# vani-nag/OWLRayTracing

Hardware: AMD Instinct MI355X
Metric: kNN queries/sec (10M pts, k=10) (higher is better)
Workload: dtype f32; 1 GPU; TrueKNN on 10000000 uniform-random 3-D points (numpy default_rng(0), [0,1)^3), k=10, start radius 0.25*(k/n)^(1/3)=0.0025; BASELINE.json configs[1]; ranks=1, n_points_total=10000000, k=10, kernel=team_kernel, parallelism=1 GPU

## Files before the change

owlraytracing_amd/csrc/lbvh.h:

```cpp
#pragma once
#include <hip/hip_runtime.h>
#include <stdint.h>

#include <string>

#include "owl/lbvh_device.h"

#define LBVH_PATH_BLOCK 64
#define LBVH_PATH_WORDS 5

namespace owlmi {

struct HipError {
  std::string what;
};
struct LbvhStateError : HipError {};

#define OWLMI_HIP(call)                                                                        \
  do {                                                                                         \
    hipError_t e_ = (call);                                                                    \
    if (e_ != hipSuccess)                                                                      \
      throw ::owlmi::HipError{std::string(#call) + " failed: " + hipGetErrorString(e_) + " (" + \
                              __FILE__ + ":" + std::to_string(__LINE__) + ")"};                \
  } while (0)

class Lbvh {
 public:
  Lbvh() = default;
  ~Lbvh();
  Lbvh(const Lbvh &) = delete;
  Lbvh &operator=(const Lbvh &) = delete;

  void build_from_points(const float *d_xyz, int64_t n, hipStream_t stream, const int32_t *d_ids = nullptr, const int32_t *d_batch = nullptr,
                         int batch_bits = 0);
  void build_from_boxes(const LbvhBox *d_boxes, int64_t n, hipStream_t stream);
  void refit_boxes(const LbvhBox *d_boxes, hipStream_t stream);

  LbvhView view() const;
  LbvhWideView wide_view() const;
  const float *scene_device() const { return scene_; }
  int32_t *nan_count() const { return reinterpret_cast<int32_t *>(scene_ + 6); }
  const int32_t *split_owner_device() const { return split_owner_; }
  const int32_t *block_paths_device() const { return point_mode_ && n_ > 1 ? block_paths_ : nullptr; }
  const int32_t *row_slot_device() const { return point_mode_ && built_ ? reinterpret_cast<const int32_t *>(order_) : nullptr; }
  const uint64_t *keys_device() const { return built_ ? codes_alt_ : nullptr; }
  int curve() const { return curve_; }
  int64_t size() const { return n_; }
  bool built() const { return built_; }
  void clear() { built_ = false; }
  bool has_points() const { return points_ != nullptr && point_mode_; }
  size_t device_bytes() const { return bytes_; }

  void download(LbvhNode *nodes, int32_t *rope_node, int32_t *rope_leaf, int32_t *prim_id,
                hipStream_t stream) const;
  void download_tables(int32_t *split_owner, int32_t *block_paths, hipStream_t stream) const;
  struct DebugInfo {
    int32_t curve, nan_count, wide_levels, wide_count[LBVH_WIDE_LEVELS];
    float scene[6];
  };
  int64_t sentinel_end() const { return (n_ + LBVH_BLOCK - 1) / LBVH_BLOCK * LBVH_BLOCK + LBVH_BLOCK; }
  void download_debug(DebugInfo *info, uint64_t *keys, LbvhPoint *points, int32_t *row_slot, LbvhBox *wide_boxes,
                      int64_t wide_capacity, hipStream_t stream) const;
  void download_boxes(LbvhBox *sorted_boxes, hipStream_t stream) const;

 private:
  void reserve(int64_t n);
  void release();
  void sort_and_tree(hipStream_t stream);
  void fit(hipStream_t stream);

  int64_t n_ = 0, cap_ = 0;
  bool built_ = false, point_mode_ = false;
  int curve_ = 0;
  size_t bytes_ = 0;
// ... 21 lines not shown
```

owlraytracing_amd/csrc/lbvh.hip:

```cpp
#include "lbvh.h"

#include "curve_key.h"

#include <hipcub/hipcub.hpp>

#include <cstdlib>
#include <cstring>

namespace owlmi {
namespace {

constexpr int kPartialBlocks = 1024;
constexpr int kBlock = 256;

struct Box6 {
  float lo[3], hi[3];
};

__device__ __forceinline__ Box6 empty_box() {
  Box6 b;
  b.lo[0] = b.lo[1] = b.lo[2] = INFINITY;
  b.hi[0] = b.hi[1] = b.hi[2] = -INFINITY;
  return b;
}
// ... 165 lines not shown
  nodes[i].other = (int32_t)j;
  split_owner[gamma] = (int32_t)i;
}

template <int SRC>
__global__ void __launch_bounds__(kBlock) table_kernel(const void *__restrict__ in, int64_t n_in,
                                                      LbvhBox *__restrict__ out, int64_t n_out) {
  int64_t j = ((int64_t)blockIdx.x * kBlock + threadIdx.x) >> 6;
  if (j >= n_out) return;
  int64_t i = j * 64 + (threadIdx.x & 63);
  Box6 b = empty_box();
  if (i < n_in) {
    if (SRC == 0) {
      LbvhPoint p = ((const LbvhPoint *)in)[i];
      float c[3] = {p.x, p.y, p.z};
      grow(b, c, c);
    } else {
      LbvhBox q = ((const LbvhBox *)in)[i];
      grow(b, q.lo, q.hi);
    }
  }
  b = wave_union(b);
  if ((threadIdx.x & 63) == 0) {
    LbvhBox o;
    for (int a = 0; a < 3; a++) {
      o.lo[a] = b.lo[a];
      o.hi[a] = b.hi[a];
    }
    out[j] = o;
  }
}

__global__ void __launch_bounds__(kBlock) block_box_kernel(const LbvhPoint *__restrict__ pts, int64_t n,
                                                          LbvhBox *__restrict__ out, int64_t n_out) {
  int64_t b = (int64_t)blockIdx.x * kBlock + threadIdx.x;
  if (b >= n_out) return;
  Box6 box = empty_box();
  for (int j = 0; j < LBVH_BLOCK; j++) {
    int64_t i = b * LBVH_BLOCK + j;
    if (i < n) {
      LbvhPoint p = pts[i];
      float c[3] = {p.x, p.y, p.z};
      grow(box, c, c);
    }
  }
  LbvhBox o;
  for (int a = 0; a < 3; a++) {
    o.lo[a] = box.lo[a];
    o.hi[a] = box.hi[a];
  }
  out[b] = o;
}

__global__ void __launch_bounds__(kBlock) block_path_kernel(const LbvhNode *__restrict__ nodes, int64_t n, int32_t *__restrict__ paths,
                                                           int64_t n_blocks) {
  const int64_t b = (int64_t)blockIdx.x * kBlock + threadIdx.x;
  if (b >= n_blocks) return;
  const int32_t lo = (int32_t)(b * LBVH_PATH_BLOCK), hi = (int32_t)((b + 1) * LBVH_PATH_BLOCK - 1 < n - 1 ? (b + 1) * LBVH_PATH_BLOCK - 1 : n - 1);
  int32_t anc[4] = {0, 0, 0, 0}, node = 0;
  for (;;) {
    const LbvhNode nd = nodes[node];
    int32_t next;
    if (hi <= nd.split) {
      if (lbvh_first(node, nd.other) == nd.split) break;
      next = nd.split;
    } else if (lo > nd.split) {
      if (lbvh_last(node, nd.other) == nd.split + 1) break;
      next = nd.split + 1;
    } else {
      break;
    }
    anc[0] = anc[1], anc[1] = anc[2], anc[2] = anc[3], anc[3] = node;
    node = next;
  }
  int32_t *out = paths + b * LBVH_PATH_WORDS;
  out[0] = anc[0], out[1] = anc[1], out[2] = anc[2], out[3] = anc[3], out[4] = node;
}

struct Pyramid {
  const LbvhPoint *points;
  const LbvhBox *boxes;
  const LbvhBox *table[4];
};

// ... 102 lines not shown
  dev_alloc(codes_alt_, (size_t)n, total);
  dev_alloc(order_, (size_t)n, total);
  dev_alloc(order_alt_, (size_t)n, total);
  sort_tmp_bytes_ = 0;
  OWLMI_HIP(hipcub::DeviceRadixSort::SortPairs(nullptr, sort_tmp_bytes_, codes_, codes_alt_, order_,
                                              order_alt_, (int)n, 0, 64, (hipStream_t)0));
  OWLMI_HIP(hipMalloc(&sort_tmp_, sort_tmp_bytes_ ? sort_tmp_bytes_ : 16));
  total += sort_tmp_bytes_;
  dev_alloc(nodes_, (size_t)(n > 1 ? n - 1 : 1), total);
  dev_alloc(split_owner_, (size_t)n, total);
  dev_alloc(rope_node_, (size_t)n, total);
  dev_alloc(rope_leaf_, (size_t)n, total);
  dev_alloc(block_paths_, ((size_t)n / LBVH_PATH_BLOCK + 1) * LBVH_PATH_WORDS, total);
  dev_alloc(points_, (size_t)n + 2 * LBVH_BLOCK, total);
  dev_alloc(boxes_, (size_t)n, total);
  dev_alloc(prim_id_, (size_t)n, total);
  int64_t m = n;
  for (int l = 0; l < 4; l++) {
    m = (m + 63) / 64;
    dev_alloc(table_[l], (size_t)m, total);
  }
  m = (n + LBVH_BLOCK - 1) / LBVH_BLOCK;
  for (int l = 0; l < LBVH_WIDE_LEVELS; l++) {
    dev_alloc(wide_[l], (size_t)m, total);
    m = (m + 63) / 64;
  }
  cap_ = n;
  bytes_ = total;
}

void Lbvh::build_wide(hipStream_t stream) {
  int64_t m = (n_ + LBVH_BLOCK - 1) / LBVH_BLOCK;
  wide_n_[0] = m;
  hipLaunchKernelGGL(block_box_kernel, dim3(blocks_for(m)), dim3(kBlock), 0, stream, points_, n_, wide_[0], m);
  OWLMI_HIP(hipGetLastError());
  wide_levels_ = 1;
  while (wide_n_[wide_levels_ - 1] > 64 && wide_levels_ < LBVH_WIDE_LEVELS) {
    const int l = wide_levels_;
    const int64_t in_n = wide_n_[l - 1], out_n = (in_n + 63) / 64;
    wide_n_[l] = out_n;
    hipLaunchKernelGGL(table_kernel<1>, dim3(blocks_for(out_n * 64)), dim3(kBlock), 0, stream,
                       (const void *)wide_[l - 1], in_n, wide_[l], out_n);
    OWLMI_HIP(hipGetLastError());
    wide_levels_++;
  }
}

LbvhWideView Lbvh::wide_view() const {
  LbvhWideView w;
  for (int l = 0; l < LBVH_WIDE_LEVELS; l++) {
    w.level[l] = l < wide_levels_ ? wide_[l] : nullptr;
    w.count[l] = l < wide_levels_ ? (int32_t)wide_n_[l] : 0;
  }
  w.levels = point_mode_ ? wide_levels_ : 0;
  return w;
}

void Lbvh::sort_and_tree(hipStream_t stream) {
  OWLMI_HIP(hipcub::DeviceRadixSort::SortPairs(sort_tmp_, sort_tmp_bytes_, codes_, codes_alt_, order_,
                                              order_alt_, (int)n_, 0, 64, stream));
  if (n_ > 1) {
    hipLaunchKernelGGL(karras_kernel, dim3(blocks_for(n_ - 1)), dim3(kBlock), 0, stream, codes_alt_, n_,
                       nodes_, split_owner_);
    OWLMI_HIP(hipGetLastError());
  }
}

// ... 158 lines not shown
```

owlraytracing_amd/csrc/trueknn.hip:

```cpp
#include "knn_thresholds.h"
#include "lane_walk.h"
#include "trueknn_engine.h"

#include <algorithm>
#include <cfloat>
#include <cmath>
#include <cstdlib>
#include <cstring>

namespace owlmi {

namespace {

constexpr int kLaneBlock = 256;

struct LaneRoundArgs {
  LbvhView bvh;
  LbvhView halo;
  int level;
  int32_t *out_level;
  float radius;
  int k;
  uint8_t *done;
  uint8_t *tie;
// ... 345 lines not shown
  boundary_valid_ = false;
  ids_given_ = d_ids != nullptr;
  if (n > state_cap_) {
    state_cap_ = 0;
    if (done_) (void)hipFree(done_);
    if (isect_sorted_) (void)hipFree(isect_sorted_);
    if (next_level_) (void)hipFree(next_level_);
    if (tie_) (void)hipFree(tie_);
    if (boundary_) (void)hipFree(boundary_);
    boundary_ = nullptr;
    tie_ = nullptr;
    done_ = nullptr;
    isect_sorted_ = nullptr;
    next_level_ = nullptr;
    try {
      OWLMI_HIP(hipMalloc((void **)&done_, (size_t)n));
      OWLMI_HIP(hipMalloc((void **)&isect_sorted_, (size_t)n * sizeof(int64_t)));
      OWLMI_HIP(hipMalloc((void **)&next_level_, (size_t)n * sizeof(int32_t)));
      OWLMI_HIP(hipMalloc((void **)&tie_, ((size_t)n + 3) & ~(size_t)3));
      OWLMI_HIP(hipMalloc((void **)&boundary_, (size_t)n));
    } catch (...) {
      bvh_.clear();
      throw;
    }
    state_cap_ = n;
  }
  try {
    bvh_.build_from_points(d_xyz, n, s, d_ids, d_batch, batch_bits);
  } catch (...) {
    bvh_.clear();
    throw;
  }
  OWLMI_HIP(hipEventRecord(ev_b_, s));
  OWLMI_HIP(hipMemcpyAsync(scene_, bvh_.scene_device(), 6 * sizeof(float), hipMemcpyDeviceToHost, s));
  OWLMI_HIP(hipStreamSynchronize(s));
  OWLMI_HIP(hipEventSynchronize(ev_b_));
  if (info) {
    float ms = 0;
    OWLMI_HIP(hipEventElapsedTime(&ms, ev_a_, ev_b_));
    info->build_ms = ms;
    info->device_bytes = (int64_t)bvh_.device_bytes();
    info->n = (int32_t)n;
  }
}

double Engine::expected_box_population(float radius) const {
  double measure = 1.0;
  int dims = 0;
  for (int a = 0; a < 3; a++) {
    const double e = (double)scene_[3 + a] - (double)scene_[a];
    if (e > 0) {
      measure *= e;
      dims++;
    }
  }
  if (dims == 0 || !(measure > 0)) return (double)bvh_.size();
  return (double)bvh_.size() / measure * std::pow(2.0 * (double)radius, dims);
}

void Engine::solve_lane(const SolveArgs &sa, tknnSolveInfo *info, hipStream_t s) { lane_rounds(sa, 0, true, info, s); }

void Engine::continue_lane(const SolveArgs &sa, int first_level, tknnSolveInfo *info, hipStream_t s) {
  lane_rounds(sa, first_level, false, info, s);
}

void Engine::lane_rounds(const SolveArgs &sa, int first_level, bool fresh, tknnSolveInfo *info, hipStream_t s) {
  const int64_t n = bvh_.size();
  const int cap = list_capacity_for(sa.k);
// ... 164 lines not shown
```

owlraytracing_amd/csrc/trueknn_engine.h:

```cpp
#pragma once
#include <hip/hip_runtime.h>
#include <stdint.h>

#include <string>
#include <type_traits>

#include "knn_device.h"
#include "lbvh.h"
#include "owlknn.h"
#include "owlknn_batch.h"
#include "owlknn_debug.h"
#include "owlknn_emst.h"
#include "owlknn_fpfh.h"
#include "owlknn_fps.h"
#include "owlknn_hdbscan.h"
#include "owlknn_icp.h"
#include "owlknn_knn.h"
#include "owlknn_meanshift.h"
#include "owlknn_nms.h"
#include "owlknn_pca.h"
#include "owlknn_periodic.h"
#include "owlknn_reduce.h"

namespace owlmi {
// ... 129 lines not shown
  int device() const { return device_; }
  int64_t size() const { return bvh_.size(); }
  const float *scene() const { return scene_; }
  const Lbvh &tree() const { return bvh_; }
  const Lbvh &halo_tree() const { return halo_; }

 private:
  struct DbCall;
  void solve_lane(const SolveArgs &sa, tknnSolveInfo *info, hipStream_t s);
  void continue_lane(const SolveArgs &sa, int first_level, tknnSolveInfo *info, hipStream_t s);
  void lane_rounds(const SolveArgs &sa, int first_level, bool fresh, tknnSolveInfo *info, hipStream_t s);
  void solve_wave(const SolveArgs &sa, tknnSolveInfo *info, hipStream_t s, bool only_unfinished = false);
  static bool wave_kernel_available();
  bool solve_team(const SolveArgs &sa, tknnSolveInfo *info, hipStream_t s);
  static bool team_kernel_supports(int k);
  static bool bigk_supports(int k);
  void solve_bigk(const SolveArgs &sa, tknnSolveInfo *info, hipStream_t s);
  void fix_ties(const SolveArgs &sa, tknnSolveInfo *info, hipStream_t s);
  void reset_stat_stripes(hipStream_t s);
  void fetch_stat_stripes(hipStream_t s);
  KernelStats fold_stat_stripes(bool with_min) const;
  void reset_solve_state(int32_t *levels, hipStream_t s);
  TeamArgs team_args(const SolveArgs &sa) const;
  void set_solve_args(TeamArgs &a, const SolveArgs &sa) const;
  tknnSolveInfo walk(const SolveArgs &sa, TeamArgs a, int nreg, const int32_t *slots, int32_t nslots, int lane_level,
                     bool count_lane_launches, hipStream_t s);
  int32_t *compact_slots(bool ties, hipStream_t s);
  void launch_tie_fix(const SolveArgs &sa, const int32_t *slots, int32_t nslots, int blocks, hipStream_t s,
                      const int32_t *d_slot_count = nullptr, int64_t expected_rows = 0);
  int first_step_estimate(const SolveArgs &sa) const;
  void *workspace(size_t bytes);
  int32_t *slot_list(int64_t n);
  float scene_[6] = {0, 0, 0, 0, 0, 0};

  int device_ = 0;
  int cu_count_ = 0;
  Lbvh bvh_;
  bool ids_given_ = false;
  int32_t num_batches_ = 0;
  int batch_bits_ = 0;
  int32_t *batch_starts_ = nullptr;
  int64_t batch_starts_cap_ = 0;
  Lbvh halo_;
  int64_t halo_n_ = 0;
  bool ignore_halo_ = false;
  int64_t halo_count() const { return ignore_halo_ ? 0 : halo_n_; }
  uint8_t *boundary_ = nullptr;
  bool boundary_valid_ = false;
  uint8_t *done_ = nullptr;
  int64_t *isect_sorted_ = nullptr;
  int32_t *next_level_ = nullptr;
  int32_t *tie_list_ = nullptr;
  uint8_t *tie_ = nullptr;
  int64_t state_cap_ = 0;
  unsigned long long *counters_ = nullptr, *h_counters_ = nullptr;
  void *wave_ws_ = nullptr;
  size_t wave_ws_bytes_ = 0;
  int db_union_resident_ = 0;
  bool wave_force_redo_ = false;
  int wave_leaf_max_ = 16;
  int32_t *slot_list_ = nullptr;
  int64_t slot_list_cap_ = 0;
  unsigned long long *halo_mask_ = nullptr;
  int64_t halo_mask_cap_ = 0;
  static size_t halo_mask_bytes(int64_t blocks);
  hipEvent_t ev_a_ = nullptr, ev_b_ = nullptr, ev_c_ = nullptr, ev_d_ = nullptr, ev_e_ = nullptr, ev_f_ = nullptr;
// ... 11 lines not shown
```

owlraytracing_amd/csrc/trueknn_team.hip:

```cpp
#include "knn_thresholds.h"
#include "team_args.h"
#include "team_lanes.h"
#include "team_walk.h"
#include "trueknn_engine.h"

#include <algorithm>
#include <cmath>
#include <cstdio>
#include <cstdlib>
#include <cstring>
#include <type_traits>

namespace owlmi {

namespace {

#ifndef TKNN_MAX_BLOCKS_3
#define TKNN_MAX_BLOCKS_3 256
#endif
#ifndef TKNN_MAX_BLOCKS_4
#define TKNN_MAX_BLOCKS_4 512
#endif
constexpr int max_blocks(int nreg) { return nreg == 4 ? TKNN_MAX_BLOCKS_4 : (nreg == 3 ? TKNN_MAX_BLOCKS_3 : 256); }
#ifndef TKNN_MAX_PER_QUERY
#define TKNN_MAX_PER_QUERY 72
#endif
#ifndef TKNN_MAX_PER_QUERY_2
#define TKNN_MAX_PER_QUERY_2 88
#endif
#ifndef TKNN_MAX_PER_QUERY_3
#define TKNN_MAX_PER_QUERY_3 88
#endif
#ifndef TKNN_MAX_PER_QUERY_4
#define TKNN_MAX_PER_QUERY_4 124
#endif
constexpr int max_per_query(int nreg) {
  return nreg == 1 ? TKNN_MAX_PER_QUERY : (nreg == 4 ? TKNN_MAX_PER_QUERY_4 : (nreg == 3 ? TKNN_MAX_PER_QUERY_3 : TKNN_MAX_PER_QUERY_2));
}
inline int lds_workgroups_per_cu(size_t lds) {
  const size_t granule = 1280, total = 160 * 1024;
  return lds ? (int)((total / granule) / ((lds + granule - 1) / granule)) : 1 << 20;
}
#ifndef TKNN_SORT_FIRST
#define TKNN_SORT_FIRST 1
#endif
#ifndef TKNN_TEAM_WAVES
#define TKNN_TEAM_WAVES 4
#endif
constexpr int kXcdCounter = kDbStats, kXcdCounterStride = 32;
constexpr int kTeamStack = 192;
constexpr int kQrecStride = 6;
constexpr int kScanBudget = 16384;
constexpr int kMaxStep = 2;
constexpr int kCountFlatGroups = 3;
constexpr int kLdsQrec = 64 * kQrecStride * 4;
constexpr int kLdsCnt = 64 * 2 * 4;
constexpr int kLdsList = 64 * 4 + 16;
constexpr int kLdsStack = kTeamStack * 4;
constexpr int kLdsShared = (kLdsCnt + kLdsList) > kLdsStack ? (kLdsCnt + kLdsList) : kLdsStack;
constexpr int kLdsSharedPadded = (kLdsShared + 15) & ~15;
constexpr int kCandCap = kCandCapacity;
template <int NREG>
struct TeamLayout {
  static constexpr int kMaxPerQuery = max_per_query(NREG);
  static constexpr int kMaxBlocks = max_blocks(NREG);
  static constexpr int kLdsBlk = kMaxBlocks * 4;
  static constexpr int kLdsMask = 64 * kMaxPerQuery;
  static constexpr int kHiWords = kMaxBlocks > 256 ? (kMaxPerQuery + 31) / 32 : 0;
  static constexpr int kLdsHi = 64 * kHiWords * 4;
  static constexpr int kEntStride = kMaxPerQuery + 4;
  static constexpr int kLdsEnt = 4 * kEntStride * 4;
  static constexpr int kLdsCand = 4 * kCandCap * 8;
  static constexpr int kOffMask = kLdsQrec + kLdsBlk;
  static constexpr int kOffHi = kOffMask + kLdsMask;
  static constexpr int kOffShared = kOffHi + kLdsHi;
  static constexpr int kOffEnt = kOffShared + kLdsSharedPadded;
  static constexpr int kOffCand = kOffEnt + kLdsEnt;
  static constexpr int kTeamLds = kOffCand + kLdsCand;
  static_assert(kEntStride % 4 == 0 && kOffEnt % 16 == 0, "entry lists must be 16-byte aligned");
  static_assert(kLdsMask % 4 == 0, "the ninth bits are words");
  static_assert(kMaxPerQuery <= 124 && kMaxPerQuery / 4 < 32, "list-length buckets of the pass lists are one bit each of a 32-bit word");
};

struct TeamLds {
  float *qrec;
  int32_t *blk;
  uint8_t *qblk;
  uint32_t *qhi;
  uint32_t *qcnt;
  int32_t *qlist;
  int32_t *ent;
  unsigned long long *cand;
};

template <bool SELECT, bool HALO, int NREG, bool FULL, bool TWO>
__device__ __forceinline__ void team_pass(const TeamArgs &a, const TeamLds &L, int n_list, int32_t first_slot,
                                          const LbvhPoint *own_pts, const LbvhPoint *halo_pts, int lane) {
  const int team = lane >> 4, tl = lane & 15;
  constexpr int kMaxPerQuery = TeamLayout<NREG>::kMaxPerQuery, kEntStride = TeamLayout<NREG>::kEntStride;
  static_assert(!(SELECT && TWO), "only a COUNT pass serves two levels");
  n_list = __builtin_amdgcn_readfirstlane(n_list);
  [[maybe_unused]] unsigned long long tp[4] = {0, 0, 0, 0};
  for (int r0 = 0; r0 < n_list; r0 += 4) {
    [[maybe_unused]] unsigned long long tp_mark = 0;
    if (TKNN_DIAG_BUILD && (a.diag & 128)) tp_mark = __builtin_amdgcn_s_memtime();
#define TP_LAP(i)                                                     \
  do {                                                                \
    if (TKNN_DIAG_BUILD && (a.diag & 128)) {                          \
      const unsigned long long now_ = __builtin_amdgcn_s_memtime();   \
      tp[i] += now_ - tp_mark;                                        \
      tp_mark = now_;                                                 \
    }                                                                 \
  } while (0)
    const bool on = r0 + team < n_list;
    int qi = 0;
    if (on) qi = L.qlist[r0 + team];
    const float *rec = L.qrec + qi * kQrecStride;
    const float t_qx = rec[0], t_qy = rec[1], t_qz = rec[2];
    const int32_t t_qid = __float_as_int(rec[3]);
    const float t_r = rec[4];
    const float t_mg = (fmaxf(fmaxf(fabsf(t_qx), fabsf(t_qy)), fabsf(t_qz)) + 2.0f * t_r) * 4.76837158203125e-07f;
    const float in_below = t_r - t_mg, in_upto = t_r + t_mg;
    const float r_inner = t_r * 0.5f;
    const float i0_below = r_inner - t_mg, i0_upto = r_inner + t_mg;
    uint32_t cnt_i0 = 0;
    const int packed = __float_as_int(rec[5]);
    [[maybe_unused]] int32_t out_row = 0;
    if (SELECT) out_row = a.bvh.prim_id[first_slot + qi];
    const int my_n = on ? (packed & 0xff) : 0;
    const int steps = max(max((int)__builtin_amdgcn_readlane(my_n, 0), (int)__builtin_amdgcn_readlane(my_n, 16)),
                          max((int)__builtin_amdgcn_readlane(my_n, 32), (int)__builtin_amdgcn_readlane(my_n, 48)));
    if (TKNN_DIAG_BUILD && (a.diag & 16) && lane == 0) atomicAdd(&a.counters[15], (unsigned long long)steps);
    const uint8_t *mine = L.qblk + qi * kMaxPerQuery;
    const int last = my_n - 1;
    const int32_t nan_block = a.wide[0].count[0];
    const int own_pos = (packed >> 8) & 0xff;
    const int n_near = (packed >> 16) & 0xff;
    const int last_near = n_near ? n_near - 1 : last;
    const int both = min(own_pos, last_near - own_pos);
    const bool right_longer = last_near - own_pos > own_pos;
    auto list_pos = [&](int it) -> int {
      if (!SELECT) return it;
      const int half = (it + 1) >> 1;
      const int alt = (it & 1) ? half : -half;
      const int far = it - both;
      const int off = it <= 2 * both ? alt : (right_longer ? far : -far);
      return it > last_near ? it : own_pos + off;
    };
    auto list_entry = [&](int pos) -> int32_t {
      int lp = list_pos(pos);
      if (n_near && lp >= n_near) lp = kMaxPerQuery - 1 - (lp - n_near);
      const int at = min(max(lp, 0), kMaxPerQuery - 1);
      int slot_at = mine[at];
      if (TeamLayout<NREG>::kHiWords) slot_at |= (int)((L.qhi[qi * TeamLayout<NREG>::kHiWords + (at >> 5)] >> (at & 31)) & 1u) << 8;
      int32_t e = L.blk[slot_at];
      if (TKNN_DIAG_BUILD && (a.diag & 64)) e = L.blk[mine[0]];
      return resolve_entry<HALO>(pos <= last ? e : nan_block);
    };
    const int steps4 = (steps + 3) & ~3;
    int32_t *my_ent = L.ent + team * kEntStride;
    for (int base = 0; base < steps4 + 4; base += 16)
      if (base + tl < kEntStride) my_ent[base + tl] = list_entry(base + tl);
    t_wave_sync();
    uint32_t cnt = 0;
    uint32_t bd[NREG], bi[NREG];
#pragma unroll
    for (int j = 0; j < NREG; j++) {
      bd[j] = 0x7f7fffffu;
      bi[j] = 0u;
    }
    constexpr bool full = FULL;
    uint32_t left_out = 0xffffffffu;
    auto kth_dist = [&]() -> float {
      uint32_t reg = bd[0];
#pragma unroll
      for (int j = 1; j < NREG; j++) reg = ((a.k - 1) >> 4) == j ? bd[j] : reg;
      return __uint_as_float(t_lane_read(reg, (team << 4) + ((a.k - 1) & 15)));
    };
    float tau2 = INFINITY;
    bool dirty = false;
    uint32_t fill_n = 0;
    auto merge_buffer = [&]() {
      t_wave_sync();
      t_merge_rows<NREG>(bd, bi, left_out, full, L.cand + team * kCandCap, fill_n, tl);
      t_wave_sync();
      fill_n = 0;
      dirty = false;
// ... 48 lines not shown
      if (__ballot(fabsf(t - t_r) <= t_mg) != 0ull) in = (t <= in_below) || ((t <= in_upto) && knn_in_box(p.x, p.y, p.z, t_r, t_qx, t_qy, t_qz));
      cnt = t_count(cnt, __ballot(in));
      bool cand = in && (p.id != t_qid);
      if (TKNN_DIAG_BUILD && (a.diag & 1)) cand = false;
      const uint32_t d2_bits = __float_as_uint(t_dist2(dx, dy, dz));
      unsigned long long *my_buf = L.cand + team * kCandCap;
      my_buf[tl] = ((unsigned long long)d2_bits << 32) | (uint32_t)p.id;
      t_wave_sync();
      t_sorted_row(d2_bits, (uint32_t)p.id, cand, tl, [&](int from) { return my_buf[from]; }, bd[0], bi[0]);
      t_wave_sync();
      tau2 = knn_gate_from_worst(kth_dist());
    };
    TP_LAP(0);
    if (!SELECT && steps <= a.count_flat_max) {
      auto flat = [&](auto groups_c) {
        constexpr int kBlocks = 4 * decltype(groups_c)::value;
        LbvhPoint c[kBlocks];
#pragma unroll
        for (int j = 0; j < kBlocks; j += 4) {
          const t_int4 g = my_groups[j >> 2];
          c[j + 0] = load_block_point<HALO>(own_pts, halo_pts, g.x, own_base, lane_bytes);
          c[j + 1] = load_block_point<HALO>(own_pts, halo_pts, g.y, own_base, lane_bytes);
          c[j + 2] = load_block_point<HALO>(own_pts, halo_pts, g.z, own_base, lane_bytes);
          c[j + 3] = load_block_point<HALO>(own_pts, halo_pts, g.w, own_base, lane_bytes);
        }
        __builtin_amdgcn_sched_barrier(0);
#pragma unroll
        for (int j = 0; j < kBlocks; j++) {
          process(c[j]);
          if (j == 3) TP_LAP(1);
        }
        if (kBlocks > 4) TP_LAP(2);
      };
      if (steps > 8)
        flat(std::integral_constant<int, 3>{});
      else if (steps > 4)
        flat(std::integral_constant<int, 2>{});
      else if (steps > 0)
        flat(std::integral_constant<int, 1>{});
    } else {
      t_point4 b0, b1, b2, b3;
      {
        const t_int4 g = my_groups[0];
        b0 = fetch(g.x);
        __builtin_amdgcn_sched_barrier(0);
        b1 = fetch(g.y);
        __builtin_amdgcn_sched_barrier(0);
        b2 = fetch(g.z);
        __builtin_amdgcn_sched_barrier(0);
        b3 = fetch(g.w);
        __builtin_amdgcn_sched_barrier(0);
      }
      for (int it = 0; it < steps; it += 4) {
        const t_int4 g = my_groups[(it >> 2) + 1];
        if (SELECT && it == 0) {
          if (NREG == 1 && TKNN_SORT_FIRST == 0)
            process(unpack(b0), true);
          else
            sort_first(unpack(b0));
        } else {
          process(unpack(b0));
        }
        b0 = fetch(g.x);
        process(unpack(b1));
        b1 = fetch(g.y);
        process(unpack(b2));
        b2 = fetch(g.z);
// ... 17 lines not shown
      v = min(v, (uint32_t)__builtin_amdgcn_update_dpp(-1, (int)v, 0x122 , 0xf, 0xf, false));
      v = min(v, (uint32_t)__builtin_amdgcn_update_dpp(-1, (int)v, 0x121 , 0xf, 0xf, false));
      left_out = v;
    }
    cnt = t_team_sum(cnt);
    const uint32_t self = cnt ? 1u : 0u;
    const uint32_t others = cnt - self;
    if (TWO) cnt_i0 = t_team_sum(cnt_i0);
    uint32_t tied = 0u;
    if (SELECT) {
      bool tie[NREG];
      bool any = false;
#pragma unroll
      for (int j = 0; j < NREG; j++) {
        uint32_t before = t_team_shr1(bd[j]);
        if (j > 0) before |= t_dpp<0x121>(bd[j - 1]) & (tl == 0 ? 0xffffffffu : 0u);
        tie[j] = ((j > 0) | (tl >= 1)) & (16 * j + tl <= a.k) & (bd[j] == before);
        if (full && j == NREG - 1) tie[j] |= (tl == 15) & (left_out == bd[j]);
        any |= tie[j];
      }
      if (__ballot(any) != 0ull) {
        const float qmax = fmaxf(fmaxf(fabsf(t_qx), fabsf(t_qy)), fabsf(t_qz));
        any = false;
        bool edge = false;
        const float q_r0 = a.start_radii ? a.start_radii[a.bvh.prim_id[first_slot + qi]] : a.start_radius;
#pragma unroll
        for (int j = 0; j < NREG; j++) {
          const bool t = tie[j] && tie_may_straddle(__uint_as_float(bd[j]), q_r0, t_r, qmax, a.tie_span);
          any |= t;
          edge |= t && (16 * j + tl == a.k || (full && j == NREG - 1 && tl == 15 && left_out == bd[j]));
        }
        if (on && edge) knn_note_tie_edge(a.tie, first_slot + qi);
      }
      tied = ((uint32_t)(__ballot(any) >> (team * 16)) & 0xffffu) ? 1u : 0u;
    }
    if (on && tl == 0) {
      uint32_t *out = L.qcnt + qi * 2;
      if (!TWO) {
        out[0] = cnt;
        out[1] = (self << 31) | (tied << 30);
      } else {
        out[0] = cnt_i0;
        out[1] = cnt | (self << 31);
      }
    }
    if (SELECT) {
      if (on && others >= (uint32_t)a.k) {
#pragma unroll
        for (int reg = 0; reg < NREG; reg++) {
          const int j = tl + 16 * reg;
          if (j >= a.k) continue;
          const int64_t o = (int64_t)out_row * a.k + j;
          const int32_t prim = knn_key_prim(((uint64_t)bd[reg] << 32) | bi[reg]);
          const float d = __uint_as_float(bd[reg]);
          if (a.out_idx) a.out_idx[o] = prim;
          if (a.out_dist) a.out_dist[o] = d;
          if (a.out_fb) {
            int2 *rec8 = (int2 *)(a.out_fb + o);
            rec8[0] = make_int2(prim, __float_as_int(d));
            rec8[1] = make_int2(j == 0 ? 0 : a.k, 0);
            if (j != 0) rec8[2] = make_int2(0, 0);
          }
        }
      }
    }
    TP_LAP(3);
  }
#undef TP_LAP
  if (TKNN_DIAG_BUILD && (a.diag & 128) && lane == 0)
    for (int i = 0; i < 4; i++) atomicAdd(&a.counters[(SELECT ? 36 : 28) + i], tp[i]);
}

template <bool HALO, int NREG, bool FULL>
__global__ void __launch_bounds__(kTeamBlock) __attribute__((amdgpu_waves_per_eu(TKNN_TEAM_WAVES))) team_kernel(TeamArgs a) {
  extern __shared__ __align__(16) unsigned char smem[];
  const int lane = threadIdx.x & 63;
  const int wid = threadIdx.x >> 6;
  const int tl = lane & 15;
  using Lay = TeamLayout<NREG>;
  constexpr int kMaxPerQuery = Lay::kMaxPerQuery;
  unsigned char *base = smem + wid * Lay::kTeamLds;
  float *qrec = (float *)base;
  int32_t *blk = (int32_t *)(base + kLdsQrec);
  uint8_t *qblk = (uint8_t *)(base + Lay::kOffMask);
  uint32_t *qhi = (uint32_t *)(base + Lay::kOffHi);
  constexpr int kMaxBlocks = Lay::kMaxBlocks;
  uint32_t *qcnt = (uint32_t *)(base + Lay::kOffShared);
  int32_t *qlist = (int32_t *)(base + Lay::kOffShared + kLdsCnt);
  int32_t *stack = (int32_t *)(base + Lay::kOffShared);
  int32_t *ent = (int32_t *)(base + Lay::kOffEnt);
  unsigned long long *cand = (unsigned long long *)(base + Lay::kOffCand);

  const LbvhPoint *own_pts = a.bvh.points + tl, *halo_pts = a.halo.points ? a.halo.points + tl : a.bvh.points + tl;
  unsigned long long my_isect_sum = 0, wave_node_tests = 0, wave_point_tests = 0;
  uint32_t my_levels = 0, my_unfinished = 0;
  int wave_levels = 0, wave_err = 0;
  uint32_t my_handed = 0;
  [[maybe_unused]] unsigned long long diag_scanned = 0, diag_listed = 0;
  int wave_min_handover = 0x7fffffff;
#if TKNN_DIAG_BUILD
  unsigned long long ph[5] = {0, 0, 0, 0, 0}, t_mark = __builtin_amdgcn_s_memtime();
#define PHASE_END(i)                                         \
  do {                                                       \
    const unsigned long long now_ = __builtin_amdgcn_s_memtime(); \
    ph[i] += now_ - t_mark;                                  \
    t_mark = now_;                                           \
  } while (0)
#else
#define PHASE_END(i) \
  do {               \
  } while (0)
#endif
// ... 314 lines not shown
        if (__ballot(active) == 0ull) break;
      }
      const int my_packed = my_nblk | (my_own_pos << 8) | (my_nblk > n_in ? n_in << 16 : n_out << 24);
      qrec[lane * kQrecStride + 5] = __int_as_float(my_packed);

      PHASE_END(1);
      const bool speculate = m == 1 && active && !served && level > 0 && prev_others * 8u >= (uint32_t)(a.k + a.k / 2);
      const bool count_first = active && !served && !speculate;
      served = false;
      auto build_qlist = [&](bool sel, int nblk) -> int {
        const int bucket = nblk >> 2;
        if (lane == 0) qlist[64] = 0;
        t_wave_sync();
        if (sel) __hip_atomic_fetch_or((uint32_t *)&qlist[64], 1u << bucket, __ATOMIC_RELAXED, __HIP_MEMORY_SCOPE_WAVEFRONT);
        t_wave_sync();
        uint32_t present = (uint32_t)__builtin_amdgcn_readfirstlane(qlist[64]);
        int base = 0, pos = 0;
        while (present) {
          const int b = __ffs((int)present) - 1;
          present &= present - 1u;
          const bool mine = sel && bucket == b;
          const unsigned long long bm = __ballot(mine);
          if (mine) pos = base + t_rank(bm);
          base += __popcll(bm);
        }
        if (sel) qlist[pos] = lane;
        t_wave_sync();
        return base;
      };
      {
        const int n_count = build_qlist(count_first, my_nblk);
        if (!(TKNN_DIAG_BUILD && (a.diag & 4))) {
          if (m > 1)
            team_pass<false, HALO, NREG, false, true>(a, L, n_count, g * 64, own_pts, halo_pts, lane);
          else
            team_pass<false, HALO, NREG, false, false>(a, L, n_count, g * 64, own_pts, halo_pts, lane);
        }
        t_wave_sync();
      }
      PHASE_END(2);
      uint32_t c0 = 0, c1 = 0, selfc = 0;
      int fin_at = -1;
      if (count_first) {
        c0 = qcnt[lane * 2 + 0];
        const uint32_t w1 = qcnt[lane * 2 + 1];
        c1 = m > 1 ? (w1 & 0x3fffffffu) : 0u;
        selfc = w1 >> 31;
        if (c0 - selfc >= (uint32_t)a.k)
          fin_at = 0;
        else if (m > 1 && c1 - selfc >= (uint32_t)a.k)
          fin_at = 1;
      }
      int sel_nblk = my_nblk;
      if (reuse && a.merge_ext && count_first && fin_at < 0 && ((m > 1 ? c1 : c0) - selfc) * 8u >= (uint32_t)(a.k + a.k / 2)) {
        fin_at = m;
        const int pk = __float_as_int(qrec[lane * kQrecStride + 5]);
        sel_nblk = (pk & 0xff) + ((pk >> 24) & 0xff);
        qrec[lane * kQrecStride + 4] = qrec[lane * kQrecStride + 4] * 2.0f;
        qrec[lane * kQrecStride + 5] = __int_as_float(sel_nblk | (pk & 0xff00) | ((pk & 0xff) << 16) | (pk & (int)0xff000000u));
      }
      const bool select_now = speculate || fin_at >= 0;
      if (m > 1 && fin_at == 0) qrec[lane * kQrecStride + 4] = r_in0;
      {
        t_wave_sync();
        const int n_select = build_qlist(select_now, sel_nblk);
        if (!(TKNN_DIAG_BUILD && (a.diag & 2))) team_pass<true, HALO, NREG, FULL, false>(a, L, n_select, g * 64, own_pts, halo_pts, lane);
        t_wave_sync();
      }
      PHASE_END(3);
      const bool ext_sel = fin_at == m;
      bool finished = fin_at >= 0 && !ext_sel;
      uint32_t last_others = prev_others;
      if (speculate) {
        c0 = qcnt[lane * 2 + 0];
        selfc = qcnt[lane * 2 + 1] >> 31;
        finished = c0 - selfc >= (uint32_t)a.k;
        fin_at = finished ? 0 : -1;
      }
      uint32_t c_ext = 0, n_back = 0;
      if (ext_sel) {
        c_ext = qcnt[lane * 2 + 0];
        finished = c_ext - selfc >= (uint32_t)a.k;
        const int pk = __float_as_int(qrec[lane * kQrecStride + 5]);
        n_back = ((uint32_t)pk >> 24) & 0xffu;
        qrec[lane * kQrecStride + 5] = __int_as_float(pk & 0x00ffffff);
      }
      int levels_run = 0;
      if (count_first || speculate) {
        levels_run = finished || ext_sel ? fin_at + 1 : m;
        isect += c0;
        if (levels_run > 1) isect += c1;
        isect += c_ext;
        my_levels += (uint32_t)levels_run;
        last_others = ext_sel ? c_ext - selfc : (m > 1 ? c1 : c0) - selfc;
        prev_others = last_others;
      }
      wave_levels = max(wave_levels, (int)t_wave_max((float)(active ? level + levels_run : 0)));
      {
        const unsigned long long passes = (count_first ? 1ull : 0ull) + (select_now ? 1ull : 0ull);
// ... 81 lines not shown
    tie[i] = 0;
  }
  if (levels)
    for (int64_t i = tid; i < n; i += nth) levels[i] = -1;
}

}

bool Engine::team_kernel_supports(int k) { return k >= 1 && k <= 64; }


int Engine::first_step_estimate(const SolveArgs &sa) const {
  float radius = sa.start_radius;
  for (int m = 1; m < 3; m++) {
    if (expected_box_population(radius) >= 0.5 * sa.k) return m;
    radius *= 2.0f;
  }
  return 3;
}

bool Engine::solve_team(const SolveArgs &sa, tknnSolveInfo *info, hipStream_t s) {
  const int64_t n = bvh_.size();
  if (n >= (1ll << 28)) return false;
  TeamArgs a = team_args(sa);
  set_solve_args(a, sa);
  a.first_step = sa.d_start_radii ? 1 : first_step_estimate(sa);
  {
    float radius = sa.start_radius;
    for (int t = 1; t < std::min(a.first_step, kMaxStep); t++) radius *= 2.0f;
    a.first_ext = !sa.d_start_radii && expected_box_population(radius) < 2.5 * sa.k ? 1 : 0;
    if (const char *e = getenv("TKNN_TEAM_EXT")) a.first_ext = atoi(e) > 0 ? a.first_ext : -1;
    a.merge_ext = 1;
    if (const char *e = getenv("TKNN_TEAM_MERGE")) a.merge_ext = atoi(e) > 0 ? 1 : 0;
    a.count_flat_max = 4 * kCountFlatGroups;
    if (const char *e = getenv("TKNN_TEAM_COUNT_FLAT")) a.count_flat_max = std::max(0, std::min(atoi(e), 4 * kCountFlatGroups));
  }
  {
    int dims = 0;
    for (int ax = 0; ax < 3; ax++) dims += scene_[3 + ax] > scene_[ax] ? 1 : 0;
    if (halo_count() > 0) dims = 3;
    a.tie_span = dims >= 3 ? 1.73206f : (dims == 2 ? 1.41422f : 1.00001f);
  }
  if (TKNN_DIAG_BUILD)
    if (const char *d = getenv("TKNN_TEAM_DIAG")) a.diag = atoi(d);
  a.ngroups = (int32_t)((n + 63) / 64);

  const int nreg = nreg_for(sa.k);
  const char *walk_all = getenv("TKNN_TEAM_WALK_ALL");
  if (sa.k > 32 && walk_all && atoi(walk_all)) {
    reset_solve_state(sa.d_levels, s);
    const tknnSolveInfo all = walk(sa, a, 4, nullptr, (int32_t)n, 0, false, s);
    if (info) *info = all;
    return true;
  }
  int per_cu = 2;
  static_assert(kDbStripes * kDbStripeWords >= 8 * kXcdCounterStride, "the packet counters borrow the words of RT-DBSCAN's striped statistics");
  const size_t lds = (size_t)kTeamBlock / 64 * (size_t)(nreg == 1 ? TeamLayout<1>::kTeamLds : (nreg == 2 ? TeamLayout<2>::kTeamLds
                                                         : (nreg == 3 ? TeamLayout<3>::kTeamLds : TeamLayout<4>::kTeamLds)));
  const bool full_list = sa.k == 16 * nreg;
  using TeamEntry = void (*)(TeamArgs);
  static const TeamEntry entries[2][4][2] = {
      {{team_kernel<false, 1, false>, team_kernel<false, 1, true>}, {team_kernel<false, 2, false>, team_kernel<false, 2, true>},
       {team_kernel<false, 3, false>, team_kernel<false, 3, true>}, {team_kernel<false, 4, false>, team_kernel<false, 4, true>}},
      {{team_kernel<true, 1, false>, team_kernel<true, 1, true>}, {team_kernel<true, 2, false>, team_kernel<true, 2, true>},
       {team_kernel<true, 3, false>, team_kernel<true, 3, true>}, {team_kernel<true, 4, false>, team_kernel<true, 4, true>}}};
  const TeamEntry entry = entries[halo_count() > 0 ? 1 : 0][nreg - 1][full_list ? 1 : 0];
  if (hipOccupancyMaxActiveBlocksPerMultiprocessor(&per_cu, (const void *)entry, kTeamBlock, lds) != hipSuccess) per_cu = 2;
  per_cu = std::max(1, std::min(per_cu, lds_workgroups_per_cu(lds)));
  if (const char *cap = getenv("TKNN_TEAM_WAVES_PER_CU"))
    per_cu = std::max(1, std::min(per_cu, atoi(cap)));
  const int64_t want = (a.ngroups + kTeamBlock / 64 - 1) / (kTeamBlock / 64);
  const int blocks = (int)std::max<int64_t>(1, std::min<int64_t>(want, (int64_t)cu_count_ * per_cu));

  hipLaunchKernelGGL(team_prep_kernel, dim3(cu_count_ * 4), dim3(256), 0, s, done_, tie_, n, counters_, sa.phase >= 2 ? nullptr : sa.d_levels);
  OWLMI_HIP(hipEventRecord(ev_a_, s));
  {
    void *kargs[] = {(void *)&a};
    OWLMI_HIP(hipLaunchKernel((const void *)entry, dim3(blocks), dim3(kTeamBlock), kargs, lds, s));
  }
  OWLMI_HIP(hipGetLastError());
  OWLMI_HIP(hipEventRecord(ev_b_, s));
  launch_tie_fix(sa, tie_list_, -1, std::min(cu_count_ * 4, kTieListCap / 4), s);
  OWLMI_HIP(hipEventRecord(ev_c_, s));
  fetch_stat_stripes(s);
  OWLMI_HIP(hipMemcpyAsync(h_counters_ + 10, counters_ + kTieCounter, 3 * sizeof(unsigned long long), hipMemcpyDeviceToHost, s));
  OWLMI_HIP(hipStreamSynchronize(s));
  const KernelStats st = fold_stat_stripes(true);
  float ms = 0;
  OWLMI_HIP(hipEventElapsedTime(&ms, ev_a_, ev_b_));
  if (st.handed_over == 0 && h_counters_[10] <= (unsigned long long)kTieListCap) {
    ties_early_ = true;
    early_tie_rows_ = (int64_t)h_counters_[10];
    early_tie_left_ = (int64_t)h_counters_[12];
    OWLMI_HIP(hipEventElapsedTime(&early_tie_ms_, ev_b_, ev_c_));
  }
#if TKNN_DIAG_BUILD
  if (getenv("TKNN_TEAM_DIAG")) {
    unsigned long long t[5];
    OWLMI_HIP(hipMemcpy(t, counters_ + 10, sizeof t, hipMemcpyDeviceToHost));
// ... 63 lines not shown
```

Measured before the change: 2.111 billion queries/s.

## Add compact team-kernel layout with smaller LDS lists for sparse uniform scenes

Adds a COMPACT variant of the team kernel for k<=16 that caps per-query block lists at 40 entries, shrinking per-wave LDS so more waves fit per CU (waves_per_eu 5), and limits the flat count pass to two groups. The host picks this layout from the expected list length at the last start radius and from a dense-block share that the block-box kernel now counts during the BVH build. This aims to raise occupancy and cut LDS pressure on uniform data. The cost is an extra atomic and memset in the build, inline-asm tweaks that steer register allocation, and a risk of list overflow or fallback when the heuristic misjudges the density.

```diff
diff --git a/owlraytracing_amd/csrc/lbvh.h b/owlraytracing_amd/csrc/lbvh.h
--- a/owlraytracing_amd/csrc/lbvh.h
+++ b/owlraytracing_amd/csrc/lbvh.h
@@ -40,6 +40,7 @@
   LbvhWideView wide_view() const;
   const float *scene_device() const { return scene_; }
   int32_t *nan_count() const { return reinterpret_cast<int32_t *>(scene_ + 6); }
+  int32_t *dense_blocks() const { return reinterpret_cast<int32_t *>(scene_ + 7); }
   const int32_t *split_owner_device() const { return split_owner_; }
   const int32_t *block_paths_device() const { return point_mode_ && n_ > 1 ? block_paths_ : nullptr; }
   const int32_t *row_slot_device() const { return point_mode_ && built_ ? reinterpret_cast<const int32_t *>(order_) : nullptr; }
diff --git a/owlraytracing_amd/csrc/lbvh.hip b/owlraytracing_amd/csrc/lbvh.hip
--- a/owlraytracing_amd/csrc/lbvh.hip
+++ b/owlraytracing_amd/csrc/lbvh.hip
@@ -221,24 +221,43 @@
 }
 
 __global__ void __launch_bounds__(kBlock) block_box_kernel(const LbvhPoint *__restrict__ pts, int64_t n,
-                                                          LbvhBox *__restrict__ out, int64_t n_out) {
+                                                          LbvhBox *__restrict__ out, int64_t n_out, const float *__restrict__ scene,
+                                                          int32_t *__restrict__ dense) {
   int64_t b = (int64_t)blockIdx.x * kBlock + threadIdx.x;
-  if (b >= n_out) return;
-  Box6 box = empty_box();
-  for (int j = 0; j < LBVH_BLOCK; j++) {
-    int64_t i = b * LBVH_BLOCK + j;
-    if (i < n) {
-      LbvhPoint p = pts[i];
-      float c[3] = {p.x, p.y, p.z};
-      grow(box, c, c);
-    }
-  }
-  LbvhBox o;
-  for (int a = 0; a < 3; a++) {
-    o.lo[a] = box.lo[a];
-    o.hi[a] = box.hi[a];
-  }
-  out[b] = o;
+  bool is_dense = false;
+  if (b < n_out) {
+    Box6 box = empty_box();
+    for (int j = 0; j < LBVH_BLOCK; j++) {
+      int64_t i = b * LBVH_BLOCK + j;
+      if (i < n) {
+        LbvhPoint p = pts[i];
+        float c[3] = {p.x, p.y, p.z};
+        grow(box, c, c);
+      }
+    }
+    LbvhBox o;
+    for (int a = 0; a < 3; a++) {
+      o.lo[a] = box.lo[a];
+      o.hi[a] = box.hi[a];
+    }
+    out[b] = o;
+    float measure = 1.f, longest = -INFINITY;
+    int dims = 0;
+    for (int a = 0; a < 3; a++) {
+      const float e = scene[3 + a] - scene[a];
+      if (e > 0.f) {
+        measure *= e;
+        dims++;
+      }
+      longest = fmaxf(longest, box.hi[a] - box.lo[a]);
+    }
+    if (dims > 0 && longest >= 0.f) {
+      const float edge = powf((float)LBVH_BLOCK * measure / (float)n, 1.0f / (float)dims);
+      is_dense = longest < 0.5f * edge;
+    }
+  }
+  const unsigned long long m = __ballot(is_dense);
+  if (m != 0ull && (threadIdx.x & 63) == 0) atomicAdd(dense, (int32_t)__popcll(m));
 }
 
 __global__ void __launch_bounds__(kBlock) block_path_kernel(const LbvhNode *__restrict__ nodes, int64_t n, int32_t *__restrict__ paths,
@@ -407,7 +426,8 @@
 void Lbvh::build_wide(hipStream_t stream) {
   int64_t m = (n_ + LBVH_BLOCK - 1) / LBVH_BLOCK;
   wide_n_[0] = m;
-  hipLaunchKernelGGL(block_box_kernel, dim3(blocks_for(m)), dim3(kBlock), 0, stream, points_, n_, wide_[0], m);
+  OWLMI_HIP(hipMemsetAsync(dense_blocks(), 0, sizeof(int32_t), stream));
+  hipLaunchKernelGGL(block_box_kernel, dim3(blocks_for(m)), dim3(kBlock), 0, stream, points_, n_, wide_[0], m, scene_, dense_blocks());
   OWLMI_HIP(hipGetLastError());
   wide_levels_ = 1;
   while (wide_n_[wide_levels_ - 1] > 64 && wide_levels_ < LBVH_WIDE_LEVELS) {
diff --git a/owlraytracing_amd/csrc/trueknn.hip b/owlraytracing_amd/csrc/trueknn.hip
--- a/owlraytracing_amd/csrc/trueknn.hip
+++ b/owlraytracing_amd/csrc/trueknn.hip
@@ -401,8 +401,15 @@
     throw;
   }
   OWLMI_HIP(hipEventRecord(ev_b_, s));
-  OWLMI_HIP(hipMemcpyAsync(scene_, bvh_.scene_device(), 6 * sizeof(float), hipMemcpyDeviceToHost, s));
+  float scene_words[8];
+  OWLMI_HIP(hipMemcpyAsync(scene_words, bvh_.scene_device(), sizeof scene_words, hipMemcpyDeviceToHost, s));
   OWLMI_HIP(hipStreamSynchronize(s));
+  std::memcpy(scene_, scene_words, sizeof scene_);
+  {
+    int32_t dense = 0;
+    std::memcpy(&dense, scene_words + 7, sizeof dense);
+    dense_block_share_ = (double)dense / (double)((n + LBVH_BLOCK - 1) / LBVH_BLOCK);
+  }
   OWLMI_HIP(hipEventSynchronize(ev_b_));
   if (info) {
     float ms = 0;
diff --git a/owlraytracing_amd/csrc/trueknn_engine.h b/owlraytracing_amd/csrc/trueknn_engine.h
--- a/owlraytracing_amd/csrc/trueknn_engine.h
+++ b/owlraytracing_amd/csrc/trueknn_engine.h
@@ -185,6 +185,7 @@
   void *workspace(size_t bytes);
   int32_t *slot_list(int64_t n);
   float scene_[6] = {0, 0, 0, 0, 0, 0};
+  double dense_block_share_ = 0;
 
   int device_ = 0;
   int cu_count_ = 0;
diff --git a/owlraytracing_amd/csrc/trueknn_team.hip b/owlraytracing_amd/csrc/trueknn_team.hip
--- a/owlraytracing_amd/csrc/trueknn_team.hip
+++ b/owlraytracing_amd/csrc/trueknn_team.hip
@@ -33,6 +33,9 @@
 #endif
 #ifndef TKNN_MAX_PER_QUERY_4
 #define TKNN_MAX_PER_QUERY_4 124
+#endif
+#ifndef TKNN_MAX_PER_QUERY_COMPACT
+#define TKNN_MAX_PER_QUERY_COMPACT 40
 #endif
 constexpr int max_per_query(int nreg) {
   return nreg == 1 ? TKNN_MAX_PER_QUERY : (nreg == 4 ? TKNN_MAX_PER_QUERY_4 : (nreg == 3 ? TKNN_MAX_PER_QUERY_3 : TKNN_MAX_PER_QUERY_2));
@@ -47,12 +50,21 @@
 #ifndef TKNN_TEAM_WAVES
 #define TKNN_TEAM_WAVES 4
 #endif
+#ifndef TKNN_TEAM_WAVES_COMPACT
+#define TKNN_TEAM_WAVES_COMPACT 5
+#endif
 constexpr int kXcdCounter = kDbStats, kXcdCounterStride = 32;
 constexpr int kTeamStack = 192;
 constexpr int kQrecStride = 6;
 constexpr int kScanBudget = 16384;
 constexpr int kMaxStep = 2;
 constexpr int kCountFlatGroups = 3;
+#ifndef TKNN_COUNT_FLAT_GROUPS_COMPACT
+#define TKNN_COUNT_FLAT_GROUPS_COMPACT 2
+#endif
+constexpr double kCompactDenseShare = 0.05;
+constexpr double kCompactMeanList = 17.4;
+constexpr int count_flat_groups(bool compact) { return compact ? TKNN_COUNT_FLAT_GROUPS_COMPACT : kCountFlatGroups; }
 constexpr int kLdsQrec = 64 * kQrecStride * 4;
 constexpr int kLdsCnt = 64 * 2 * 4;
 constexpr int kLdsList = 64 * 4 + 16;
@@ -60,9 +72,10 @@
 constexpr int kLdsShared = (kLdsCnt + kLdsList) > kLdsStack ? (kLdsCnt + kLdsList) : kLdsStack;
 constexpr int kLdsSharedPadded = (kLdsShared + 15) & ~15;
 constexpr int kCandCap = kCandCapacity;
-template <int NREG>
+template <int NREG, bool COMPACT = false>
 struct TeamLayout {
-  static constexpr int kMaxPerQuery = max_per_query(NREG);
+  static_assert(!COMPACT || NREG == 1, "the compact layout is for one list register per lane");
+  static constexpr int kMaxPerQuery = COMPACT ? TKNN_MAX_PER_QUERY_COMPACT : max_per_query(NREG);
   static constexpr int kMaxBlocks = max_blocks(NREG);
   static constexpr int kLdsBlk = kMaxBlocks * 4;
   static constexpr int kLdsMask = 64 * kMaxPerQuery;
@@ -80,6 +93,7 @@
   static_assert(kEntStride % 4 == 0 && kOffEnt % 16 == 0, "entry lists must be 16-byte aligned");
   static_assert(kLdsMask % 4 == 0, "the ninth bits are words");
   static_assert(kMaxPerQuery <= 124 && kMaxPerQuery / 4 < 32, "list-length buckets of the pass lists are one bit each of a 32-bit word");
+  static_assert(!COMPACT || kTeamLds <= 6 * 1280, "the compact layout is six LDS granules per wave");
 };
 
 struct TeamLds {
@@ -93,11 +107,12 @@
   unsigned long long *cand;
 };
 
-template <bool SELECT, bool HALO, int NREG, bool FULL, bool TWO>
+template <bool SELECT, bool HALO, int NREG, bool FULL, bool TWO, bool COMPACT>
 __device__ __forceinline__ void team_pass(const TeamArgs &a, const TeamLds &L, int n_list, int32_t first_slot,
                                           const LbvhPoint *own_pts, const LbvhPoint *halo_pts, int lane) {
   const int team = lane >> 4, tl = lane & 15;
-  constexpr int kMaxPerQuery = TeamLayout<NREG>::kMaxPerQuery, kEntStride = TeamLayout<NREG>::kEntStride;
+  using Lay = TeamLayout<NREG, COMPACT>;
+  constexpr int kMaxPerQuery = Lay::kMaxPerQuery, kEntStride = Lay::kEntStride;
   static_assert(!(SELECT && TWO), "only a COUNT pass serves two levels");
   n_list = __builtin_amdgcn_readfirstlane(n_list);
   [[maybe_unused]] unsigned long long tp[4] = {0, 0, 0, 0};
@@ -152,7 +167,7 @@
       if (n_near && lp >= n_near) lp = kMaxPerQuery - 1 - (lp - n_near);
       const int at = min(max(lp, 0), kMaxPerQuery - 1);
       int slot_at = mine[at];
-      if (TeamLayout<NREG>::kHiWords) slot_at |= (int)((L.qhi[qi * TeamLayout<NREG>::kHiWords + (at >> 5)] >> (at & 31)) & 1u) << 8;
+      if (Lay::kHiWords) slot_at |= (int)((L.qhi[qi * Lay::kHiWords + (at >> 5)] >> (at & 31)) & 1u) << 8;
       int32_t e = L.blk[slot_at];
       if (TKNN_DIAG_BUILD && (a.diag & 64)) e = L.blk[mine[0]];
       return resolve_entry<HALO>(pos <= last ? e : nan_block);
@@ -267,7 +282,7 @@
         }
         if (kBlocks > 4) TP_LAP(2);
       };
-      if (steps > 8)
+      if (count_flat_groups(COMPACT) >= 3 && steps > 8)
         flat(std::integral_constant<int, 3>{});
       else if (steps > 4)
         flat(std::integral_constant<int, 2>{});
@@ -351,7 +366,9 @@
         }
         if (on && edge) knn_note_tie_edge(a.tie, first_slot + qi);
       }
-      tied = ((uint32_t)(__ballot(any) >> (team * 16)) & 0xffffu) ? 1u : 0u;
+      int team_here = team;
+      if (COMPACT) asm volatile("" : "+v"(team_here));
+      tied = ((uint32_t)(__ballot(any) >> (team_here * 16)) & 0xffffu) ? 1u : 0u;
     }
     if (on && tl == 0) {
       uint32_t *out = L.qcnt + qi * 2;
@@ -378,7 +395,9 @@
             int2 *rec8 = (int2 *)(a.out_fb + o);
             rec8[0] = make_int2(prim, __float_as_int(d));
             rec8[1] = make_int2(j == 0 ? 0 : a.k, 0);
-            if (j != 0) rec8[2] = make_int2(0, 0);
+            int nought = 0;
+            if (COMPACT) asm volatile("v_mov_b32 %0, 0" : "=v"(nought));
+            if (j != 0) rec8[2] = make_int2(nought, nought);
           }
         }
       }
@@ -390,13 +409,14 @@
     for (int i = 0; i < 4; i++) atomicAdd(&a.counters[(SELECT ? 36 : 28) + i], tp[i]);
 }
 
-template <bool HALO, int NREG, bool FULL>
-__global__ void __launch_bounds__(kTeamBlock) __attribute__((amdgpu_waves_per_eu(TKNN_TEAM_WAVES))) team_kernel(TeamArgs a) {
+template <bool HALO, int NREG, bool FULL, bool COMPACT>
+__global__ void __launch_bounds__(kTeamBlock) __attribute__((amdgpu_waves_per_eu(COMPACT ? TKNN_TEAM_WAVES_COMPACT : TKNN_TEAM_WAVES)))
+team_kernel(TeamArgs a) {
   extern __shared__ __align__(16) unsigned char smem[];
   const int lane = threadIdx.x & 63;
   const int wid = threadIdx.x >> 6;
   const int tl = lane & 15;
-  using Lay = TeamLayout<NREG>;
+  using Lay = TeamLayout<NREG, COMPACT>;
   constexpr int kMaxPerQuery = Lay::kMaxPerQuery;
   unsigned char *base = smem + wid * Lay::kTeamLds;
   float *qrec = (float *)base;
@@ -777,9 +797,9 @@
         const int n_count = build_qlist(count_first, my_nblk);
         if (!(TKNN_DIAG_BUILD && (a.diag & 4))) {
           if (m > 1)
-            team_pass<false, HALO, NREG, false, true>(a, L, n_count, g * 64, own_pts, halo_pts, lane);
+            team_pass<false, HALO, NREG, false, true, COMPACT>(a, L, n_count, g * 64, own_pts, halo_pts, lane);
           else
-            team_pass<false, HALO, NREG, false, false>(a, L, n_count, g * 64, own_pts, halo_pts, lane);
+            team_pass<false, HALO, NREG, false, false, COMPACT>(a, L, n_count, g * 64, own_pts, halo_pts, lane);
         }
         t_wave_sync();
       }
@@ -809,7 +829,7 @@
       {
         t_wave_sync();
         const int n_select = build_qlist(select_now, sel_nblk);
-        if (!(TKNN_DIAG_BUILD && (a.diag & 2))) team_pass<true, HALO, NREG, FULL, false>(a, L, n_select, g * 64, own_pts, halo_pts, lane);
+        if (!(TKNN_DIAG_BUILD && (a.diag & 2))) team_pass<true, HALO, NREG, FULL, false, COMPACT>(a, L, n_select, g * 64, own_pts, halo_pts, lane);
         t_wave_sync();
       }
       PHASE_END(3);
@@ -957,8 +977,45 @@
     if (const char *e = getenv("TKNN_TEAM_EXT")) a.first_ext = atoi(e) > 0 ? a.first_ext : -1;
     a.merge_ext = 1;
     if (const char *e = getenv("TKNN_TEAM_MERGE")) a.merge_ext = atoi(e) > 0 ? 1 : 0;
-    a.count_flat_max = 4 * kCountFlatGroups;
-    if (const char *e = getenv("TKNN_TEAM_COUNT_FLAT")) a.count_flat_max = std::max(0, std::min(atoi(e), 4 * kCountFlatGroups));
+  }
+  const int nreg = nreg_for(sa.k);
+  bool compact = false;
+  {
+    float r_last = sa.start_radius;
+    for (int t = 1; t < std::min(a.first_step, kMaxStep) + (a.first_ext > 0 ? 1 : 0); t++) r_last *= 2.0f;
+    double measure = 1.0, mean_list = 0;
+    int dims = 0;
+    for (int ax = 0; ax < 3; ax++) {
+      const double e = (double)scene_[3 + ax] - (double)scene_[ax];
+      if (e > 0) measure *= e, dims++;
+    }
+    if (dims > 0) mean_list = std::pow(1.0 + 2.0 * (double)r_last / std::pow((double)LBVH_BLOCK * measure / (double)n, 1.0 / dims), dims);
+    const char *why = "the lists are expected to fit";
+    if (nreg != 1)
+      why = "k > 16";
+    else if (sa.d_start_radii)
+      why = "per-query start radii";
+    else if (halo_count() > 0)
+      why = "a halo tree";
+    else if (dims == 0)
+      why = "a scene without extent";
+    else if (dense_block_share_ > kCompactDenseShare)
+      why = "dense blocks";
+    else if (mean_list > kCompactMeanList)
+      why = "long lists expected";
+    else
+      compact = true;
+    if (const char *e = getenv("TKNN_TEAM_LAYOUT")) {
+      if (nreg == 1 && !sa.d_start_radii && !strcmp(e, "compact")) compact = true, why = "TKNN_TEAM_LAYOUT";
+      if (!strcmp(e, "roomy")) compact = false, why = "TKNN_TEAM_LAYOUT";
+    }
+    if (getenv("TKNN_VERBOSE"))
+      fprintf(stderr, "[team] layout %s (%s): k %d, dense-block share %.4f, %.1f blocks per list expected at radius %.5g\n",
+              compact ? "compact" : "roomy", why, sa.k, dense_block_share_, mean_list, (double)r_last);
+  }
+  {
+    a.count_flat_max = 4 * count_flat_groups(compact);
+    if (const char *e = getenv("TKNN_TEAM_COUNT_FLAT")) a.count_flat_max = std::max(0, std::min(atoi(e), 4 * count_flat_groups(compact)));
   }
   {
     int dims = 0;
@@ -970,7 +1027,6 @@
     if (const char *d = getenv("TKNN_TEAM_DIAG")) a.diag = atoi(d);
   a.ngroups = (int32_t)((n + 63) / 64);
 
-  const int nreg = nreg_for(sa.k);
   const char *walk_all = getenv("TKNN_TEAM_WALK_ALL");
   if (sa.k > 32 && walk_all && atoi(walk_all)) {
     reset_solve_state(sa.d_levels, s);
@@ -980,16 +1036,19 @@
   }
   int per_cu = 2;
   static_assert(kDbStripes * kDbStripeWords >= 8 * kXcdCounterStride, "the packet counters borrow the words of RT-DBSCAN's striped statistics");
-  const size_t lds = (size_t)kTeamBlock / 64 * (size_t)(nreg == 1 ? TeamLayout<1>::kTeamLds : (nreg == 2 ? TeamLayout<2>::kTeamLds
+  const size_t lds = (size_t)kTeamBlock / 64 * (size_t)(nreg == 1 ? (compact ? TeamLayout<1, true>::kTeamLds : TeamLayout<1>::kTeamLds)
+                                                         : (nreg == 2 ? TeamLayout<2>::kTeamLds
                                                          : (nreg == 3 ? TeamLayout<3>::kTeamLds : TeamLayout<4>::kTeamLds)));
   const bool full_list = sa.k == 16 * nreg;
   using TeamEntry = void (*)(TeamArgs);
   static const TeamEntry entries[2][4][2] = {
-      {{team_kernel<false, 1, false>, team_kernel<false, 1, true>}, {team_kernel<false, 2, false>, team_kernel<false, 2, true>},
-       {team_kernel<false, 3, false>, team_kernel<false, 3, true>}, {team_kernel<false, 4, false>, team_kernel<false, 4, true>}},
-      {{team_kernel<true, 1, false>, team_kernel<true, 1, true>}, {team_kernel<true, 2, false>, team_kernel<true, 2, true>},
-       {team_kernel<true, 3, false>, team_kernel<true, 3, true>}, {team_kernel<true, 4, false>, team_kernel<true, 4, true>}}};
-  const TeamEntry entry = entries[halo_count() > 0 ? 1 : 0][nreg - 1][full_list ? 1 : 0];
+      {{team_kernel<false, 1, false, false>, team_kernel<false, 1, true, false>}, {team_kernel<false, 2, false, false>, team_kernel<false, 2, true, false>},
+       {team_kernel<false, 3, false, false>, team_kernel<false, 3, true, false>}, {team_kernel<false, 4, false, false>, team_kernel<false, 4, true, false>}},
+      {{team_kernel<true, 1, false, false>, team_kernel<true, 1, true, false>}, {team_kernel<true, 2, false, false>, team_kernel<true, 2, true, false>},
+       {team_kernel<true, 3, false, false>, team_kernel<true, 3, true, false>}, {team_kernel<true, 4, false, false>, team_kernel<true, 4, true, false>}}};
+  static const TeamEntry compact_entries[2][2] = {{team_kernel<false, 1, false, true>, team_kernel<false, 1, true, true>},
+                                                  {team_kernel<true, 1, false, true>, team_kernel<true, 1, true, true>}};
+  const TeamEntry entry = compact ? compact_entries[halo_count() > 0 ? 1 : 0][full_list ? 1 : 0] : entries[halo_count() > 0 ? 1 : 0][nreg - 1][full_list ? 1 : 0];
   if (hipOccupancyMaxActiveBlocksPerMultiprocessor(&per_cu, (const void *)entry, kTeamBlock, lds) != hipSuccess) per_cu = 2;
   per_cu = std::max(1, std::min(per_cu, lds_workgroups_per_cu(lds)));
   if (const char *cap = getenv("TKNN_TEAM_WAVES_PER_CU"))
```

After: 2.109 billion queries/s. No clear change (-0.1%).
